# zero-savvy/vimz

Measured on AMD Instinct MI355X. Metric: nova_folding_steps_per_sec, higher is better.
Workload: dtype u32 limbs (256-bit Montgomery integers over BN254 Fr/Fq)

## Files before the change

### include/vimz_hip_testing.h

```cpp
#ifndef VIMZ_HIP_TESTING_H
#define VIMZ_HIP_TESTING_H
#include "vimz_hip.h"

#ifdef __cplusplus
extern "C" {
#endif

int vimz_cf_poke(vimz_cf* v, int which, size_t index, const uint64_t value[4]);
int vimz_cf_selfcheck(int steps, uint32_t* result, uint64_t counts[8]);
int64_t vimz_cf_selfcheck_last_step(int steps, void* buf, size_t cap);
int64_t vimz_cf_selfcheck_merge(int segs_run0, int segs_run1, void* buf, size_t cap);
int64_t vimz_worker_selftest(int jobs);
int vimz_strict_bits_selfcheck(int field, int values, uint64_t out[8]);
void vimz_test_forge_public_slot(int on);
int vimz_decider_selfcheck(int steps, int full, uint32_t* result, uint64_t counts[4]);
int vimz_testing_kzg_setup_seeded(vimz_ctx* ctx, const uint8_t* seed, size_t seed_len, size_t n, vimz_bases** srs_out, uint64_t vk_g2_out[16]);
int vimz_testing_decider_setup_seeded(vimz_cf* prover, const uint64_t kzg_vk_g2[16], int light, const uint8_t* seed, size_t seed_len, vimz_decider** out, double seconds[4]);

int vimz_test_fp29_probe(vimz_ctx* ctx, int field, int op, const uint32_t* a, const uint32_t* b, const uint32_t* c, const uint32_t* d, uint32_t* out, size_t n);
int vimz_test_spmv_cross16(vimz_ctx* ctx, const vimz_r1cs* S, size_t row0, size_t nrows, const vimz_vec* z, vimz_vec* az, vimz_vec* bz, vimz_vec* cz,
                           const vimz_vec* az1, const vimz_vec* bz1, const vimz_vec* cz1, const uint64_t u1[4], const uint64_t u2[4], int form, vimz_vec* T);
int vimz_test_cross_term_masked(vimz_ctx* ctx, size_t n, const vimz_vec* az1, const vimz_vec* bz1, const vimz_vec* cz1, const uint64_t u1[4], const vimz_vec* az2,
                                const vimz_vec* bz2, const vimz_vec* cz2, const uint64_t u2[4], int form, vimz_vec* T, vimz_vec* Tm, size_t nb);

#ifdef __cplusplus
}
#endif
#endif
```

### vimz_amd/csrc/image_hash.hip

```cpp
#include <hip/hip_runtime.h>
#include <algorithm>
#include <atomic>
#include <chrono>
#include <cstring>
#include <mutex>
#include <thread>
#include <vector>

#include "internal.hpp"
#include "fp29.hpp"
#include "circuit/poseidon_params.hpp"

using namespace vz;

namespace {

typedef Fp29<BnFr> F29;
constexpr int IH_STRIDE = 12;
constexpr int IH_WAVE = 64;
constexpr uint32_t IH_MAX_LEN = 1u << 20;

struct IhTables {
  const uint32_t* c[10]; const uint32_t* m[10]; const uint32_t* s[10]; const uint32_t* f[10];
  uint32_t rp[10];
};
struct IhImage { const uint8_t* px; const uint32_t* units; uint32_t h, w, ch, block, L, pad; };
struct IhSeg { uint32_t first_block, n_chains, chain_off, L; };
struct IhChain { uint32_t img, unit; };

__device__ __forceinline__ F29 ih_load29(const uint32_t* __restrict__ base, size_t idx) {
  const uint4* q = reinterpret_cast<const uint4*>(base + (size_t)IH_STRIDE * idx);
  const uint4 a = q[0], b = q[1], c = q[2];
  F29 r; r.v[0] = a.x; r.v[1] = a.y; r.v[2] = a.z; r.v[3] = a.w; r.v[4] = b.x; r.v[5] = b.y; r.v[6] = b.z; r.v[7] = b.w; r.v[8] = c.x;
  return r;
}
__device__ __forceinline__ F29 ih_shfl29(const F29& v, int src_lane) {
  F29 r;
#pragma unroll
  for (int k = 0; k < 9; k++) r.v[k] = __shfl(v.v[k], src_lane);
  return r;
}

__device__ __forceinline__ F29 ih_element(const IhImage& I, uint32_t unit, uint32_t e) {
  uint32_t w8[8] = {0, 0, 0, 0, 0, 0, 0, 0};
  if (I.units) {
    const uint4* q = reinterpret_cast<const uint4*>(I.units + 8 * ((size_t)unit * I.L + e));
    const uint4 a = q[0], b = q[1];
    w8[0] = a.x; w8[1] = a.y; w8[2] = a.z; w8[3] = a.w; w8[4] = b.x; w8[5] = b.y; w8[6] = b.z; w8[7] = b.w;
  } else {
    uint32_t row, col0, run;
    if (!I.block) {
      row = unit; col0 = e * 10; run = I.w - col0;
    } else {
      const uint32_t bw = (I.w + I.block - 1) / I.block, per_row = (I.block + 9) / 10;
      const uint32_t br = unit / bw, bc = unit % bw, r = e / per_row, c = e % per_row;
      row = br * I.block + r; col0 = bc * I.block + c * 10;
      const uint32_t end = min(I.w, (bc + 1) * I.block);
      run = row < I.h && col0 < end ? end - col0 : 0;
    }
    const uint32_t nc = I.ch < 3 ? I.ch : 3;
    const uint8_t* p = I.px + ((size_t)row * I.w + col0) * I.ch;
#pragma unroll
    for (uint32_t k = 0; k < 10; k++)
#pragma unroll
      for (uint32_t c = 0; c < 3; c++) {
        const uint32_t byte = 3 * k + c;
        if (k < run && c < nc) w8[byte >> 2] |= (uint32_t)p[(size_t)k * I.ch + c] << (8 * (byte & 3));
      }
  }
  F29 r2;
#pragma unroll
  for (int i = 0; i < 9; i++) r2.v[i] = F29::R2_29.l[i];
  return F29::mul(F29::pack(w8), r2);
}

template <int T>
__device__ __forceinline__ F29 ih_perm(const IhTables& P, F29 s, uint32_t li, int lane_base, int G) {
  const uint32_t* __restrict__ PC = P.c[T];
  const uint32_t* __restrict__ PM = P.m[T];
  const uint32_t* __restrict__ PS = P.s[T];
  const uint32_t* __restrict__ PF = P.f[T];
  const uint32_t rp = P.rp[T];
  const bool mine = li < (uint32_t)T;
  F29 Mrow[T];
#pragma unroll
  for (int j = 0; j < T; j++) Mrow[j] = mine ? ih_load29(PM, (size_t)li * T + j) : F29::zero();
  auto full_round = [&](uint32_t r) {
    if (mine) {
      s = F29::add(s, ih_load29(PC, (size_t)r * T + li));
      const F29 x2 = F29::sqr(s), x4 = F29::sqr(x2);
      s = F29::mul(x4, s);
    }
    F29 prod[T];
#pragma unroll
    for (int j = 0; j < T; j++) prod[j] = F29::mul(Mrow[j], ih_shfl29(s, lane_base + j));
#pragma unroll
    for (int stride = 1; stride < T; stride <<= 1)
#pragma unroll
      for (int j = 0; j + stride < T; j += 2 * stride) prod[j] = F29::add(prod[j], prod[j + stride]);
    s = prod[0].weak_reduce();
  };
  for (uint32_t r = 0; r < 4; r++) full_round(r);
  const bool l0 = li == 0;
  F29 ct = F29::zero(), rw = F29::zero(), cl = F29::zero();
  if (mine) { const size_t q = 3 * (size_t)li; ct = ih_load29(PS, q); rw = ih_load29(PS, q + 1); cl = ih_load29(PS, q + 2); }
  for (uint32_t r = 0; r < rp; r++) {
    F29 ctn = F29::zero(), rwn = F29::zero(), cln = F29::zero();
    if (mine && r + 1 < rp) { const size_t q = 3 * ((size_t)(r + 1) * T + li); ctn = ih_load29(PS, q); rwn = ih_load29(PS, q + 1); cln = ih_load29(PS, q + 2); }
    s = F29::add(s, ct);
    const F29 sl0 = ih_shfl29(s, lane_base);
    const F29 m1 = F29::mul(l0 ? s : rw, s);
    const F29 u = F29::mul(l0 ? rw : cl, sl0);
    F29 x4 = F29::zero();
    if (l0) x4 = F29::sqr(m1);
    const F29 x4b = ih_shfl29(x4, lane_base);
    const F29 m2 = F29::mul(x4b, u);
    F29 p = l0 ? m2 : (mine ? m1 : F29::zero());
    for (int off = G >> 1; off >= 1; off >>= 1) {
      F29 o;
#pragma unroll
      for (int k = 0; k < 9; k++) o.v[k] = __shfl_xor(p.v[k], off);
      p = F29::add(p, o);
    }
    s = (l0 ? p : (mine ? F29::add(s, m2) : s)).weak_reduce();
    ct = ctn; rw = rwn; cl = cln;
  }
  {
    F29 acc = F29::zero();
#pragma unroll
    for (int j = 0; j < T - 1; j++) {
      const F29 sj = ih_shfl29(s, lane_base + 1 + j);
      if (mine && !l0) acc = F29::add(acc, F29::mul(ih_load29(PF, (size_t)(li - 1) * (T - 1) + j), sj));
    }
    if (mine && !l0) s = acc.weak_reduce();
  }
  for (uint32_t r = 4 + rp; r < 8 + rp; r++) full_round(r);
  return s;
}

__global__ void __launch_bounds__(IH_WAVE) k_image_digests(IhTables P, const IhImage* __restrict__ imgs, const IhSeg* __restrict__ segs, uint32_t n_segs,
                                                           const IhChain* __restrict__ chains, uint32_t* __restrict__ out) {
  uint32_t sg = 0;
  while (sg + 1 < n_segs && blockIdx.x >= segs[sg + 1].first_block) sg++;
  const IhSeg S = segs[sg];
  const int G = S.L >= 8 ? 16 : 8;
  const uint32_t li = threadIdx.x & (uint32_t)(G - 1);
  const int lane_base = (int)(threadIdx.x & ~(uint32_t)(G - 1));
  const uint32_t k = (blockIdx.x - S.first_block) * (IH_WAVE / G) + threadIdx.x / G;
  const bool live = k < S.n_chains;
  const IhChain C = chains[S.chain_off + (live ? k : 0)];
  const IhImage I = imgs[C.img];
  const uint32_t L = S.L, rounds = (L + 7) / 8;
  F29 h = F29::zero();
  uint32_t done = 0;
  for (uint32_t r = 0; r < rounds; r++) {
    const uint32_t kin = r == 0 ? min(L, 8u) : min(L - done, 7u);
    const uint32_t t = r == 0 ? kin + 1 : kin + 2;
    F29 s = F29::zero();
    if (li >= 1 && li < t) s = (r > 0 && li == 1) ? h : ih_element(I, C.unit, done + li - (r == 0 ? 1 : 2));
    switch (t) {
      case 2: s = ih_perm<2>(P, s, li, lane_base, G); break;
      case 3: s = ih_perm<3>(P, s, li, lane_base, G); break;
      case 4: s = ih_perm<4>(P, s, li, lane_base, G); break;
      case 5: s = ih_perm<5>(P, s, li, lane_base, G); break;
      case 6: s = ih_perm<6>(P, s, li, lane_base, G); break;
      case 7: s = ih_perm<7>(P, s, li, lane_base, G); break;
      case 8: s = ih_perm<8>(P, s, li, lane_base, G); break;
      default: s = ih_perm<9>(P, s, li, lane_base, G); break;
    }
    h = ih_shfl29(s, lane_base);
    done += kin;
  }
  if (live && li == 0) {
    F29 one = F29::zero(); one.v[0] = 1;
    const F29 x = F29::mul(h, one).canon();
    uint32_t w8[8]; x.unpack(w8);
    uint4* o = reinterpret_cast<uint4*>(out + 8 * (size_t)k + 8 * (size_t)S.chain_off);
    o[0] = make_uint4(w8[0], w8[1], w8[2], w8[3]); o[1] = make_uint4(w8[4], w8[5], w8[6], w8[7]);
  }
}

struct IhHostTables { std::vector<uint32_t> words; size_t c[10], m[10], s[10], f[10]; uint32_t rp[10]; };
const IhHostTables& ih_host_tables() {
  static const IhHostTables T = [] {
    IhHostTables H{};
    auto put = [&](const std::vector<cb::Fe>& v) {
      const size_t at = H.words.size();
      H.words.resize(at + v.size() * (size_t)IH_STRIDE, 0u);
      for (size_t i = 0; i < v.size(); i++) { const F29 x = F29::from_std(v[i]); for (int k = 0; k < 9; k++) H.words[at + i * IH_STRIDE + k] = x.v[k]; }
      return at;
    };
    for (int t = 2; t <= 9; t++) {
      const cb::PoseidonTable& P = cb::poseidon_table(t);
      const auto& S = cb::poseidon_sparse_t<BnFr>(t);
      std::vector<cb::Fe> packed((size_t)P.rp * t * 3);
      for (int r = 0; r < P.rp; r++)
        for (int i = 0; i < t; i++) {
          cb::Fe* q = &packed[3 * ((size_t)r * t + i)];
          q[0] = S.ctil[(size_t)r * t + i]; q[1] = S.row[(size_t)r * t + i]; q[2] = i ? S.col[(size_t)r * (t - 1) + i - 1] : cb::Fe::zero();
        }
      H.c[t] = put(P.C); H.m[t] = put(P.M); H.s[t] = put(packed); H.f[t] = put(S.Pfin); H.rp[t] = (uint32_t)P.rp;
    }
    return H;
  }();
  return T;
}

inline size_t ih_align(size_t x) { return (x + 255) & ~(size_t)255; }

bool ih_below_modulus(const uint64_t* x) {
  const uint32_t* m = BnFr::MOD.w;
  for (int i = 3; i >= 0; i--) {
    const uint64_t mi = (uint64_t)m[2 * i] | (uint64_t)m[2 * i + 1] << 32;
    if (x[i] != mi) return x[i] < mi;
  }
  return false;
}

}

static int fail(vimz_ctx* c, int code, const char* what, hipError_t e = hipSuccess) { return vz::vz_fail(c, code, what, e); }

// ... 165 lines not shown
```

### vimz_amd/csrc/r1cs_capi.hip

```cpp
#include <hip/hip_runtime.h>
#include <array>
#include <cstring>
#include <memory>
#include <new>
#include <unordered_map>
#include <vector>

#include "internal.hpp"
#include "r1cs_ops.hpp"

using namespace vz;

struct vimz_r1cs {
  int field = 0;
  size_t nrows = 0, ncols = 0, nnz[3] = {0, 0, 0};
  CsrDev M[3] = {};
  uint32_t* dict = nullptr; size_t ndict = 0;
  uint32_t* long_items = nullptr; uint32_t n_long = 0, n_med = 0;
  uint32_t* scratch = nullptr;
  std::vector<void*> owned;
};

#define R_TRY(x) do { hipError_t _e = (x); if (_e != hipSuccess) return vz_fail(ctx, VIMZ_ERR_HIP, #x, _e); } while (0)

// ... 199 lines not shown
  uint32_t bad[2];
  R_TRY(hipMemcpyAsync(bad, bad_d, 8, hipMemcpyDeviceToHost, s));
  R_TRY(hipStreamSynchronize(s));
  *bad_rows = bad[0];
  if (first_bad) *first_bad = bad[0] ? bad[1] : ~0ull;
  return VIMZ_OK;
}

int vimz_vec_axpy(vimz_ctx* ctx, vimz_vec* x1, const uint64_t r[4], int form, const vimz_vec* x2, size_t n) {
  if (!ctx || !x1 || !x2 || !r) return vz_fail(ctx, VIMZ_ERR_INVALID, "vimz_vec_axpy: bad argument");
  if (x1->field != x2->field || n > x1->n || n > x2->n) return vz_fail(ctx, VIMZ_ERR_INVALID, "vimz_vec_axpy: fields differ or a vector is shorter than n");
  if (x1 == x2) return vz_fail(ctx, VIMZ_ERR_INVALID, "vimz_vec_axpy: x1 and x2 must be different vectors");
  if (!n) return VIMZ_OK;
  std::lock_guard<std::mutex> g(ctx->mu);
  R_TRY(hipSetDevice(ctx->device));
  int rc = field_dispatch(x1->field, [&](auto f) {
    typedef decltype(f) F;
    F a; memcpy(a.v, r, 32);
    if (!a.is_reduced()) return vz_fail(ctx, VIMZ_ERR_INVALID, "vimz_vec_axpy: r not below the modulus");
    if (form == VIMZ_FORM_CANONICAL) a = F::to_mont(a);
    hipLaunchKernelGGL(k_axpy_inplace<F>, dim3(stream_grid(n)), dim3(256), 0, ctx->stream, n, x1->d, a, (const uint32_t*)x2->d);
    return VIMZ_OK;
  });
  if (rc) return rc;
  R_TRY(hipGetLastError());
  return VIMZ_OK;
}

}

#ifdef VIMZ_TESTING
#include "../../include/vimz_hip_testing.h"
#include "fp29_probe.hpp"

namespace {
template <class P>
__global__ void __launch_bounds__(256) k_fp29_probe(int op, const uint32_t* __restrict__ a, const uint32_t* __restrict__ b, const uint32_t* __restrict__ c,
                                                    const uint32_t* __restrict__ d, uint32_t* __restrict__ out, size_t n) {
  VZ_GRID_STRIDE(i, n) {
    uint32_t x[4][FP29_PROBE_WORDS], r[FP29_PROBE_WORDS];
    for (int k = 0; k < FP29_PROBE_WORDS; k++) { x[0][k] = a[FP29_PROBE_WORDS * i + k]; x[1][k] = b[FP29_PROBE_WORDS * i + k]; x[2][k] = c[FP29_PROBE_WORDS * i + k]; x[3][k] = d[FP29_PROBE_WORDS * i + k]; }
    fp29_probe<P>(op, x[0], x[1], x[2], x[3], r);
    for (int k = 0; k < FP29_PROBE_WORDS; k++) out[FP29_PROBE_WORDS * i + k] = r[k];
  }
}
template <class F>
int scalar_arg(vimz_ctx* ctx, const uint64_t* u, int form, F* out, const char* what) {
  memcpy(out->v, u, 32);
  if (!out->is_reduced()) return vz_fail(ctx, VIMZ_ERR_INVALID, what);
  if (form == VIMZ_FORM_CANONICAL) *out = F::to_mont(*out);
  return VIMZ_OK;
}
}

extern "C" {

int vimz_test_fp29_probe(vimz_ctx* ctx, int field, int op, const uint32_t* a, const uint32_t* b, const uint32_t* c, const uint32_t* d, uint32_t* out, size_t n) {
  if (!ctx || !a || !b || !c || !d || !out || field < 0 || field > 3) return vz_fail(ctx, VIMZ_ERR_INVALID, "vimz_test_fp29_probe: bad argument");
  {
    uint32_t zero[FP29_PROBE_WORDS] = {}, r[FP29_PROBE_WORDS];
    if (fp29_probe<BnFr>(op, zero, zero, zero, zero, r)) return vz_fail(ctx, VIMZ_ERR_INVALID, "vimz_test_fp29_probe: unknown operation");
  }
  if (!n) return VIMZ_OK;
  std::lock_guard<std::mutex> g(ctx->mu);
  R_TRY(hipSetDevice(ctx->device));
  const size_t bytes = 4 * (size_t)FP29_PROBE_WORDS * n;
  uint32_t* buf = nullptr;
  R_TRY(hipMalloc((void**)&buf, 5 * bytes));
  const uint32_t* src[4] = {a, b, c, d};
  hipError_t e = hipSuccess;
  for (int k = 0; k < 4 && e == hipSuccess; k++) e = hipMemcpyAsync((char*)buf + k * bytes, src[k], bytes, hipMemcpyHostToDevice, ctx->stream);
  if (e == hipSuccess) {
    uint32_t* p = buf; const size_t w = (size_t)FP29_PROBE_WORDS * n;
    fp29_probe_field(field, [&](auto pp) {
      typedef decltype(pp) P;
      hipLaunchKernelGGL(k_fp29_probe<P>, dim3(stream_grid(n)), dim3(256), 0, ctx->stream, op, (const uint32_t*)p, (const uint32_t*)(p + w), (const uint32_t*)(p + 2 * w), (const uint32_t*)(p + 3 * w), p + 4 * w, n);
      return 0;
    });
    e = hipGetLastError();
  }
  if (e == hipSuccess) e = hipMemcpyAsync(out, (char*)buf + 4 * bytes, bytes, hipMemcpyDeviceToHost, ctx->stream);
  const hipError_t e2 = hipStreamSynchronize(ctx->stream);
  hipFree(buf);
  if (e != hipSuccess) return vz_fail(ctx, VIMZ_ERR_HIP, "vimz_test_fp29_probe", e);
  if (e2 != hipSuccess) return vz_fail(ctx, VIMZ_ERR_HIP, "vimz_test_fp29_probe: synchronize", e2);
  return VIMZ_OK;
}

int vimz_test_spmv_cross16(vimz_ctx* ctx, const vimz_r1cs* S, size_t row0, size_t nrows, const vimz_vec* z, vimz_vec* az, vimz_vec* bz, vimz_vec* cz,
                           const vimz_vec* az1, const vimz_vec* bz1, const vimz_vec* cz1, const uint64_t u1[4], const uint64_t u2[4], int form, vimz_vec* T) {
  if (!ctx || !S || !z || !az || !bz || !cz || !u1 || !u2) return vz_fail(ctx, VIMZ_ERR_INVALID, "vimz_test_spmv_cross16: bad argument");
  if (az1 && (!bz1 || !cz1 || !T)) return vz_fail(ctx, VIMZ_ERR_INVALID, "vimz_test_spmv_cross16: a running instance needs all of az1, bz1, cz1 and T");
  if (row0 > S->nrows || nrows > S->nrows - row0) return vz_fail(ctx, VIMZ_ERR_INVALID, "vimz_test_spmv_cross16: rows outside the shape");
  const vimz_vec* vs[7] = {az, bz, cz, az1, bz1, cz1, T};
  for (const vimz_vec* v : vs) if (v && (v->field != S->field || v->n < S->nrows)) return vz_fail(ctx, VIMZ_ERR_INVALID, "vimz_test_spmv_cross16: field or length of a vector does not fit the shape");
  if (z->field != S->field || z->n < S->ncols) return vz_fail(ctx, VIMZ_ERR_INVALID, "vimz_test_spmv_cross16: z does not fit the shape");
  if (!nrows) return VIMZ_OK;
  std::lock_guard<std::mutex> g(ctx->mu);
  R_TRY(hipSetDevice(ctx->device));
  int rc = field_dispatch(S->field, [&](auto f) {
    typedef decltype(f) F;
    F a, b; int r;
    if ((r = scalar_arg(ctx, u1, form, &a, "vimz_test_spmv_cross16: u1 not below the modulus")) || (r = scalar_arg(ctx, u2, form, &b, "vimz_test_spmv_cross16: u2 not below the modulus"))) return r;
    hipLaunchKernelGGL(k_spmv_cross16<F>, dim3((unsigned)((16 * nrows + 255) / 256)), dim3(256), 0, ctx->stream, S->M[0], S->M[1], S->M[2], (const uint32_t*)S->dict, (uint32_t)row0, (uint32_t)nrows,
                       (const uint32_t*)z->d, az->d, bz->d, cz->d, az1 ? (const uint32_t*)az1->d : (const uint32_t*)nullptr, bz1 ? (const uint32_t*)bz1->d : (const uint32_t*)nullptr,
                       cz1 ? (const uint32_t*)cz1->d : (const uint32_t*)nullptr, a, b, T ? T->d : (uint32_t*)nullptr);
    return VIMZ_OK;
  });
  if (rc) return rc;
  R_TRY(hipGetLastError());
  R_TRY(hipStreamSynchronize(ctx->stream));
  return VIMZ_OK;
}

int vimz_test_cross_term_masked(vimz_ctx* ctx, size_t n, const vimz_vec* az1, const vimz_vec* bz1, const vimz_vec* cz1, const uint64_t u1[4], const vimz_vec* az2, const vimz_vec* bz2,
                                const vimz_vec* cz2, const uint64_t u2[4], int form, vimz_vec* T, vimz_vec* Tm, size_t nb) {
  if (!ctx || !az1 || !bz1 || !cz1 || !az2 || !bz2 || !cz2 || !u1 || !u2 || !T) return vz_fail(ctx, VIMZ_ERR_INVALID, "vimz_test_cross_term_masked: bad argument");
  const vimz_vec* vs[8] = {az1, bz1, cz1, az2, bz2, cz2, T, Tm};
  for (const vimz_vec* v : vs) if (v && (v->field != T->field || v->n < n)) return vz_fail(ctx, VIMZ_ERR_INVALID, "vimz_test_cross_term_masked: field or length of a vector");
  if (nb > n || n >= (1ull << 32)) return vz_fail(ctx, VIMZ_ERR_INVALID, "vimz_test_cross_term_masked: nb beyond n");
  if (T == Tm) return vz_fail(ctx, VIMZ_ERR_INVALID, "vimz_test_cross_term_masked: T and Tm must differ");
// ... 20 lines not shown
```

### vimz_amd/csrc/witness.hpp

```cpp
#pragma once
#include <hip/hip_runtime.h>
#include "fp.hpp"
#include "fp29.hpp"
#include "circuit/program.hpp"
#include "vecops.hpp"

namespace vz {

typedef Fp<BnFr> Fr;

struct WitnessDev {
  const DecompGroup* decomp; uint32_t n_decomp;
  const LaneGroup* groups; uint32_t n_groups;
  const LaneInstr* instr;
  const LaneRow* rows;
  const HashJob* jobs; uint32_t n_jobs;
  const Chain* chains; uint32_t n_chains;
  const FieldOp* fops; uint32_t n_fops;
  const LcTerm* lc_terms; const uint32_t* dict;
  const uint32_t* pc3; const uint32_t* pm3;
  const uint32_t* pc9; const uint32_t* pm9;
  const uint32_t* ps3; const uint32_t* pf3;
  const uint32_t* ps9; const uint32_t* pf9;
  uint32_t rp3, rp9;
  const uint32_t *pc3_29, *pm3_29, *ps3_29, *pf3_29, *pc9_29, *pm9_29, *ps9_29, *pf9_29;
  uint32_t poseidon29;
  uint32_t n_wires, len_z, n_priv;
};

__device__ __forceinline__ Fr fr_from_small(long long v) {
  Fr x = Fr::zero();
  unsigned long long m = v < 0 ? (unsigned long long)(-v) : (unsigned long long)v;
  x.v[0] = (uint32_t)m; x.v[1] = (uint32_t)(m >> 32);
  x = Fr::to_mont(x);
  return v < 0 ? Fr::neg(x) : x;
}
// ... 200 lines not shown
    if (mine && r + 1 < rp) { const size_t q = 3 * ((size_t)(r + 1) * T + li); ctn = load_fe<Fr>(PS, q); rwn = load_fe<Fr>(PS, q + 1); cln = load_fe<Fr>(PS, q + 2); }
    s = Fr::add(s, ct);
    const Fr sl0 = shfl_fe(s, lane_base);
    const Fr m1 = Fr::mul(l0 ? s : rw, s);
    const Fr u = Fr::mul(l0 ? rw : cl, sl0);
    Fr x4 = Fr::zero();
    if (l0) { x4 = Fr::sqr(m1); if (live && Zrow) emit(nf0 + 3 * T + r, m1, x4, Fr::mul(x4, s)); }
    const Fr x4b = shfl_fe(x4, lane_base);
    const Fr m2 = Fr::mul(x4b, u);
    Fr p = l0 ? m2 : (mine ? m1 : Fr::zero());
#pragma unroll
    for (int off = 8; off >= 1; off >>= 1) {
      Fr o;
#pragma unroll
      for (int k = 0; k < 8; k++) o.v[k] = __shfl_xor(p.v[k], off);
      p = Fr::add(p, o);
    }
    s = l0 ? p : (mine ? Fr::add(s, m2) : s);
    ct = ctn; rw = rwn; cl = cln;
  }
  {
    Fr acc = Fr::zero();
#pragma unroll
    for (int j = 0; j < T - 1; j++) {
      const Fr sj = shfl_fe(s, lane_base + 1 + j);
      if (mine && !l0) acc = Fr::add(acc, Fr::mul(load_fe<Fr>(PF, (size_t)(li - 1) * (T - 1) + j), sj));
    }
    if (mine && !l0) s = acc;
  }
  for (uint32_t r = 4 + rp; r < R; r++) full_round(r);
  return s;
}

typedef Fp29<BnFr> F29;
constexpr int F29_STRIDE = 12;
__device__ __forceinline__ F29 load29(const uint32_t* __restrict__ base, size_t idx) {
  const uint4* q = reinterpret_cast<const uint4*>(base + (size_t)F29_STRIDE * idx);
  const uint4 a = q[0], b = q[1], c = q[2];
  F29 r; r.v[0] = a.x; r.v[1] = a.y; r.v[2] = a.z; r.v[3] = a.w; r.v[4] = b.x; r.v[5] = b.y; r.v[6] = b.z; r.v[7] = b.w; r.v[8] = c.x;
  return r;
}
__device__ __forceinline__ F29 shfl29(const F29& v, int src_lane) {
  F29 r;
#pragma unroll
  for (int k = 0; k < 9; k++) r.v[k] = __shfl(v.v[k], src_lane);
  return r;
}
static_assert(F29::KNUM == 169u, "the bounds in poseidon_group29 are written for BN254 Fr's quotient estimate");
__device__ __forceinline__ F29 weak_reduce29(const F29& a) { return a.weak_reduce(); }
__device__ __forceinline__ void store29_raw(uint32_t* __restrict__ Zrow, uint32_t wire, const F29& x) {
  uint32_t w[8]; x.unpack(w);
  uint4* q = reinterpret_cast<uint4*>(Zrow + 8 * (size_t)wire);
  q[0] = make_uint4(w[0], w[1], w[2], w[3]); q[1] = make_uint4(w[4], w[5], w[6], w[7]);
}

template <int T>
__device__ __forceinline__ F29 poseidon_group29(const WitnessDev& P, const HashJob& J, bool live, F29 s, bool in_const, uint32_t li, int lane_base,
                                                uint32_t* __restrict__ Zrow) {
  const uint32_t* PC = T == 3 ? P.pc3_29 : P.pc9_29;
  const uint32_t* PM = T == 3 ? P.pm3_29 : P.pm9_29;
  const uint32_t* PS = T == 3 ? P.ps3_29 : P.ps9_29;
  const uint32_t* PF = T == 3 ? P.pf3_29 : P.pf9_29;
  const uint32_t rp = T == 3 ? P.rp3 : P.rp9;
  const uint32_t R = 8 + rp;
  const bool mine = li < (uint32_t)T;
  F29 Mrow[T];
#pragma unroll
  for (int j = 0; j < T; j++) Mrow[j] = mine ? load29(PM, (size_t)li * T + j) : F29::zero();
  const unsigned long long nf_mask = __ballot(live && li >= 1 && mine && !in_const);
  const uint32_t grp_mask16 = (uint32_t)((nf_mask >> lane_base) & 0xffffull);
  const uint32_t nf_before = __popc(grp_mask16 & ((1u << li) - 1u));
  const uint32_t nf0 = __popc(grp_mask16);
  const uint32_t elim_slot = 3 * (nf0 + 3 * T + rp + 3 * T) + 2;
  const bool bound = J.out_wire != 0;
  auto emit = [&](uint32_t index, const F29& x2, const F29& x4, const F29& x5) {
    const uint32_t slot = 3 * index;
    auto wire_of = [&](uint32_t sl) { return J.wire_base + sl - ((bound && sl > elim_slot) ? 1u : 0u); };
    store29_raw(Zrow, wire_of(slot), x2);
    store29_raw(Zrow, wire_of(slot + 1), x4);
    if (!(bound && slot + 2 == elim_slot)) store29_raw(Zrow, wire_of(slot + 2), x5);
  };
  auto full_round = [&](uint32_t r) {
    if (mine) {
      s = F29::add(s, load29(PC, (size_t)r * T + li));
      const F29 x2 = F29::sqr(s), x4 = F29::sqr(x2), x5 = F29::mul(x4, s);
      const bool folded = r == 0 && in_const;
      if (live && !folded && Zrow) {
        uint32_t index;
        if (r == 0) index = nf_before;
        else if (r < 4) index = nf0 + (r - 1) * T + li;
        else index = nf0 + 3 * T + rp + (r - 4 - rp) * T + li;
        emit(index, x2, x4, x5);
      }
      s = x5;
    }
    F29 prod[T];
#pragma unroll
    for (int j = 0; j < T; j++) prod[j] = F29::mul(Mrow[j], shfl29(s, lane_base + j));
#pragma unroll
    for (int stride = 1; stride < T; stride <<= 1)
#pragma unroll
      for (int j = 0; j + stride < T; j += 2 * stride) prod[j] = F29::add(prod[j], prod[j + stride]);
    s = weak_reduce29(prod[0]);
  };
  for (uint32_t r = 0; r < 4; r++) full_round(r);
  const bool l0 = li == 0;
  F29 ct = F29::zero(), rw = F29::zero(), cl = F29::zero();
  if (mine) { const size_t q = 3 * (size_t)li; ct = load29(PS, q); rw = load29(PS, q + 1); cl = load29(PS, q + 2); }
  for (uint32_t r = 0; r < rp; r++) {
    F29 ctn = F29::zero(), rwn = F29::zero(), cln = F29::zero();
    if (mine && r + 1 < rp) { const size_t q = 3 * ((size_t)(r + 1) * T + li); ctn = load29(PS, q); rwn = load29(PS, q + 1); cln = load29(PS, q + 2); }
    s = F29::add(s, ct);
    const F29 sl0 = shfl29(s, lane_base);
    const F29 m1 = F29::mul(l0 ? s : rw, s);
    const F29 u = F29::mul(l0 ? rw : cl, sl0);
    F29 x4 = F29::zero();
    if (l0) { x4 = F29::sqr(m1); if (live && Zrow) emit(nf0 + 3 * T + r, m1, x4, F29::mul(x4, s)); }
    const F29 x4b = shfl29(x4, lane_base);
    const F29 m2 = F29::mul(x4b, u);
    F29 p = l0 ? m2 : (mine ? m1 : F29::zero());
#pragma unroll
    for (int off = 8; off >= 1; off >>= 1) {
      F29 o;
#pragma unroll
      for (int k = 0; k < 9; k++) o.v[k] = __shfl_xor(p.v[k], off);
      p = F29::add(p, o);
    }
    s = weak_reduce29(l0 ? p : (mine ? F29::add(s, m2) : s));
    ct = ctn; rw = rwn; cl = cln;
  }
  {
    F29 acc = F29::zero();
#pragma unroll
    for (int j = 0; j < T - 1; j++) {
      const F29 sj = shfl29(s, lane_base + 1 + j);
      if (mine && !l0) acc = F29::add(acc, F29::mul(load29(PF, (size_t)(li - 1) * (T - 1) + j), sj));
    }
    if (mine && !l0) s = weak_reduce29(acc);
  }
  for (uint32_t r = 4 + rp; r < R; r++) full_round(r);
  return s;
}

static __global__ void __launch_bounds__(64) k_wit_chains(WitnessDev P, uint32_t phase, uint32_t* __restrict__ Z, uint32_t* __restrict__ job_out,
                                                   const uint32_t* __restrict__ priv_rows) {
  const uint32_t row = blockIdx.y;
  const uint32_t sub = threadIdx.x >> 4, li = threadIdx.x & 15;
  const int lane_base = (int)(threadIdx.x & ~15u);
  uint32_t want = blockIdx.x * 4 + sub, seen = 0, cid = 0xffffffffu;
  for (uint32_t c = 0; c < P.n_chains; c++) if (P.chains[c].phase == phase) { if (seen == want) { cid = c; break; } seen++; }
  const bool active_chain = cid != 0xffffffffu;
  uint32_t* Zrow = priv_rows ? nullptr : Z + 8 * (size_t)row * P.n_wires;
  const uint32_t* prow = priv_rows ? priv_rows + 8 * (size_t)row * P.n_priv : nullptr;
  uint32_t* jrow = job_out + 8 * (size_t)row * (P.n_jobs + P.n_fops);
  const uint32_t njobs = active_chain ? P.chains[cid].job_cnt : 0;
  uint32_t max_jobs = njobs;
  for (int off = 32; off >= 16; off >>= 1) max_jobs = max(max_jobs, (uint32_t)__shfl_xor((int)max_jobs, off));
  Fr prev_out = Fr::zero();
  if (P.poseidon29) {
    F29 prev29 = F29::zero();
    for (uint32_t k = 0; k < max_jobs; k++) {
      const bool live = k < njobs;
      HashJob J;
      if (live) J = P.jobs[P.chains[cid].job_off + k]; else { J.t = 3; J.wire_base = 0; J.out_wire = 0; }
      const uint32_t t = J.t;
      F29 s = F29::zero();
      bool in_const = true;
      if (live && li >= 1 && li < t) {
        const ValRef ref = J.in[li - 1];
        in_const = ref.kind == REF_CONST_ZERO;
        if (ref.kind == REF_JOB && k > 0 && ref.idx == P.chains[cid].job_off + k - 1) s = prev29;
        else s = F29::from_std(wit_value(P, ref, Zrow, jrow, prow));
      }
      const bool any9 = __any(live && t == 9), any3 = __any(live && t != 9);
      F29 out = F29::zero();
      if (any9) { F29 o = poseidon_group29<9>(P, J, live && t == 9, s, in_const, li, lane_base, Zrow); if (t == 9) out = o; }
      if (any3) { F29 o = poseidon_group29<3>(P, J, live && t == 3, s, in_const, li, lane_base, Zrow); if (t != 9) out = o; }
      prev29 = shfl29(out, lane_base);
      if (live && li == 0) {
        const Fr o = out.to_std();
        store_fe(jrow, P.chains[cid].job_off + k, o);
        if (J.out_wire && Zrow) store_fe(Zrow, J.out_wire, o);
      }
    }
    return;
  }
  for (uint32_t k = 0; k < max_jobs; k++) {
    const bool live = k < njobs;
    HashJob J;
    if (live) J = P.jobs[P.chains[cid].job_off + k]; else { J.t = 3; J.wire_base = 0; J.out_wire = 0; }
    const uint32_t t = J.t;
    Fr s = Fr::zero();
    bool in_const = true;
    if (live && li >= 1 && li < t) {
      const ValRef ref = J.in[li - 1];
      in_const = ref.kind == REF_CONST_ZERO;
      if (ref.kind == REF_JOB && k > 0 && ref.idx == P.chains[cid].job_off + k - 1) s = prev_out;
      else s = wit_value(P, ref, Zrow, jrow, prow);
    }
    const bool any9 = __any(live && t == 9), any3 = __any(live && t != 9);
    Fr out = Fr::zero();
    if (any9) { Fr o = poseidon_group<9>(P, J, live && t == 9, s, in_const, li, lane_base, Zrow); if (t == 9) out = o; }
    if (any3) { Fr o = poseidon_group<3>(P, J, live && t == 3, s, in_const, li, lane_base, Zrow); if (t != 9) out = o; }
    prev_out = shfl_fe(out, lane_base);
    if (live && li == 0) {
      store_fe(jrow, P.chains[cid].job_off + k, out);
      if (J.out_wire && Zrow) store_fe(Zrow, J.out_wire, out);
    }
  }
}

// ... 75 lines not shown
```

Before: 1369.

## Share Poseidon29 permutation using DPP broadcasts and lazy-reduced dot products

Pulls the 29-bit-limb Poseidon permutation out of the image-hash and witness-chain kernels into one shared header. The MDS row products now accumulate in 64-bit columns and run a single Montgomery reduction per dot of up to six terms, where before each product was reduced separately. Lane broadcasts and group reductions use DPP row operations in place of ds_bpermute shuffles, and the group size is now a template parameter. The DPP control encodings (row_newbcast and similar) are tied to specific hardware and add correctness risk, and the partial-round emit path is restructured.

```diff
diff --git a/include/vimz_hip_testing.h b/include/vimz_hip_testing.h
--- a/include/vimz_hip_testing.h
+++ b/include/vimz_hip_testing.h
@@ -18,6 +18,7 @@
 int vimz_testing_decider_setup_seeded(vimz_cf* prover, const uint64_t kzg_vk_g2[16], int light, const uint8_t* seed, size_t seed_len, vimz_decider** out, double seconds[4]);
 
 int vimz_test_fp29_probe(vimz_ctx* ctx, int field, int op, const uint32_t* a, const uint32_t* b, const uint32_t* c, const uint32_t* d, uint32_t* out, size_t n);
+int vimz_test_fp29_dot(vimz_ctx* ctx, int field, int K, const uint32_t* xs, const uint32_t* ys, uint32_t* out, size_t n);
 int vimz_test_spmv_cross16(vimz_ctx* ctx, const vimz_r1cs* S, size_t row0, size_t nrows, const vimz_vec* z, vimz_vec* az, vimz_vec* bz, vimz_vec* cz,
                            const vimz_vec* az1, const vimz_vec* bz1, const vimz_vec* cz1, const uint64_t u1[4], const uint64_t u2[4], int form, vimz_vec* T);
 int vimz_test_cross_term_masked(vimz_ctx* ctx, size_t n, const vimz_vec* az1, const vimz_vec* bz1, const vimz_vec* cz1, const uint64_t u1[4], const vimz_vec* az2,
diff --git a/vimz_amd/csrc/image_hash.hip b/vimz_amd/csrc/image_hash.hip
--- a/vimz_amd/csrc/image_hash.hip
+++ b/vimz_amd/csrc/image_hash.hip
@@ -9,14 +9,13 @@
 
 #include "internal.hpp"
 #include "fp29.hpp"
+#include "poseidon29.hpp"
 #include "circuit/poseidon_params.hpp"
 
 using namespace vz;
 
 namespace {
 
-typedef Fp29<BnFr> F29;
-constexpr int IH_STRIDE = 12;
 constexpr int IH_WAVE = 64;
 constexpr uint32_t IH_MAX_LEN = 1u << 20;
 
@@ -27,19 +26,6 @@
 struct IhImage { const uint8_t* px; const uint32_t* units; uint32_t h, w, ch, block, L, pad; };
 struct IhSeg { uint32_t first_block, n_chains, chain_off, L; };
 struct IhChain { uint32_t img, unit; };
-
-__device__ __forceinline__ F29 ih_load29(const uint32_t* __restrict__ base, size_t idx) {
-  const uint4* q = reinterpret_cast<const uint4*>(base + (size_t)IH_STRIDE * idx);
-  const uint4 a = q[0], b = q[1], c = q[2];
-  F29 r; r.v[0] = a.x; r.v[1] = a.y; r.v[2] = a.z; r.v[3] = a.w; r.v[4] = b.x; r.v[5] = b.y; r.v[6] = b.z; r.v[7] = b.w; r.v[8] = c.x;
-  return r;
-}
-__device__ __forceinline__ F29 ih_shfl29(const F29& v, int src_lane) {
-  F29 r;
-#pragma unroll
-  for (int k = 0; k < 9; k++) r.v[k] = __shfl(v.v[k], src_lane);
-  return r;
-}
 
 __device__ __forceinline__ F29 ih_element(const IhImage& I, uint32_t unit, uint32_t e) {
   uint32_t w8[8] = {0, 0, 0, 0, 0, 0, 0, 0};
@@ -74,68 +60,9 @@
   return F29::mul(F29::pack(w8), r2);
 }
 
-template <int T>
-__device__ __forceinline__ F29 ih_perm(const IhTables& P, F29 s, uint32_t li, int lane_base, int G) {
-  const uint32_t* __restrict__ PC = P.c[T];
-  const uint32_t* __restrict__ PM = P.m[T];
-  const uint32_t* __restrict__ PS = P.s[T];
-  const uint32_t* __restrict__ PF = P.f[T];
-  const uint32_t rp = P.rp[T];
-  const bool mine = li < (uint32_t)T;
-  F29 Mrow[T];
-#pragma unroll
-  for (int j = 0; j < T; j++) Mrow[j] = mine ? ih_load29(PM, (size_t)li * T + j) : F29::zero();
-  auto full_round = [&](uint32_t r) {
-    if (mine) {
-      s = F29::add(s, ih_load29(PC, (size_t)r * T + li));
-      const F29 x2 = F29::sqr(s), x4 = F29::sqr(x2);
-      s = F29::mul(x4, s);
-    }
-    F29 prod[T];
-#pragma unroll
-    for (int j = 0; j < T; j++) prod[j] = F29::mul(Mrow[j], ih_shfl29(s, lane_base + j));
-#pragma unroll
-    for (int stride = 1; stride < T; stride <<= 1)
-#pragma unroll
-      for (int j = 0; j + stride < T; j += 2 * stride) prod[j] = F29::add(prod[j], prod[j + stride]);
-    s = prod[0].weak_reduce();
-  };
-  for (uint32_t r = 0; r < 4; r++) full_round(r);
-  const bool l0 = li == 0;
-  F29 ct = F29::zero(), rw = F29::zero(), cl = F29::zero();
-  if (mine) { const size_t q = 3 * (size_t)li; ct = ih_load29(PS, q); rw = ih_load29(PS, q + 1); cl = ih_load29(PS, q + 2); }
-  for (uint32_t r = 0; r < rp; r++) {
-    F29 ctn = F29::zero(), rwn = F29::zero(), cln = F29::zero();
-    if (mine && r + 1 < rp) { const size_t q = 3 * ((size_t)(r + 1) * T + li); ctn = ih_load29(PS, q); rwn = ih_load29(PS, q + 1); cln = ih_load29(PS, q + 2); }
-    s = F29::add(s, ct);
-    const F29 sl0 = ih_shfl29(s, lane_base);
-    const F29 m1 = F29::mul(l0 ? s : rw, s);
-    const F29 u = F29::mul(l0 ? rw : cl, sl0);
-    F29 x4 = F29::zero();
-    if (l0) x4 = F29::sqr(m1);
-    const F29 x4b = ih_shfl29(x4, lane_base);
-    const F29 m2 = F29::mul(x4b, u);
-    F29 p = l0 ? m2 : (mine ? m1 : F29::zero());
-    for (int off = G >> 1; off >= 1; off >>= 1) {
-      F29 o;
-#pragma unroll
-      for (int k = 0; k < 9; k++) o.v[k] = __shfl_xor(p.v[k], off);
-      p = F29::add(p, o);
-    }
-    s = (l0 ? p : (mine ? F29::add(s, m2) : s)).weak_reduce();
-    ct = ctn; rw = rwn; cl = cln;
-  }
-  {
-    F29 acc = F29::zero();
-#pragma unroll
-    for (int j = 0; j < T - 1; j++) {
-      const F29 sj = ih_shfl29(s, lane_base + 1 + j);
-      if (mine && !l0) acc = F29::add(acc, F29::mul(ih_load29(PF, (size_t)(li - 1) * (T - 1) + j), sj));
-    }
-    if (mine && !l0) s = acc.weak_reduce();
-  }
-  for (uint32_t r = 4 + rp; r < 8 + rp; r++) full_round(r);
-  return s;
+template <int G, int T>
+__device__ __forceinline__ F29 ih_perm(const IhTables& P, const F29& s, uint32_t li) {
+  return poseidon29_perm<G, T>(P29Tables{P.c[T], P.m[T], P.s[T], P.f[T], P.rp[T]}, s, li, P29NoEmit{});
 }
 
 __global__ void __launch_bounds__(IH_WAVE) k_image_digests(IhTables P, const IhImage* __restrict__ imgs, const IhSeg* __restrict__ segs, uint32_t n_segs,
@@ -145,7 +72,6 @@
   const IhSeg S = segs[sg];
   const int G = S.L >= 8 ? 16 : 8;
   const uint32_t li = threadIdx.x & (uint32_t)(G - 1);
-  const int lane_base = (int)(threadIdx.x & ~(uint32_t)(G - 1));
   const uint32_t k = (blockIdx.x - S.first_block) * (IH_WAVE / G) + threadIdx.x / G;
   const bool live = k < S.n_chains;
   const IhChain C = chains[S.chain_off + (live ? k : 0)];
@@ -158,17 +84,29 @@
     const uint32_t t = r == 0 ? kin + 1 : kin + 2;
     F29 s = F29::zero();
     if (li >= 1 && li < t) s = (r > 0 && li == 1) ? h : ih_element(I, C.unit, done + li - (r == 0 ? 1 : 2));
-    switch (t) {
-      case 2: s = ih_perm<2>(P, s, li, lane_base, G); break;
-      case 3: s = ih_perm<3>(P, s, li, lane_base, G); break;
-      case 4: s = ih_perm<4>(P, s, li, lane_base, G); break;
-      case 5: s = ih_perm<5>(P, s, li, lane_base, G); break;
-      case 6: s = ih_perm<6>(P, s, li, lane_base, G); break;
-      case 7: s = ih_perm<7>(P, s, li, lane_base, G); break;
-      case 8: s = ih_perm<8>(P, s, li, lane_base, G); break;
-      default: s = ih_perm<9>(P, s, li, lane_base, G); break;
-    }
-    h = ih_shfl29(s, lane_base);
+    if (G == 16) {
+      switch (t) {
+        case 3: s = ih_perm<16, 3>(P, s, li); break;
+        case 4: s = ih_perm<16, 4>(P, s, li); break;
+        case 5: s = ih_perm<16, 5>(P, s, li); break;
+        case 6: s = ih_perm<16, 6>(P, s, li); break;
+        case 7: s = ih_perm<16, 7>(P, s, li); break;
+        case 8: s = ih_perm<16, 8>(P, s, li); break;
+        default: s = ih_perm<16, 9>(P, s, li); break;
+      }
+      h = p29_bcast<16, 0>(s);
+    } else {
+      switch (t) {
+        case 2: s = ih_perm<8, 2>(P, s, li); break;
+        case 3: s = ih_perm<8, 3>(P, s, li); break;
+        case 4: s = ih_perm<8, 4>(P, s, li); break;
+        case 5: s = ih_perm<8, 5>(P, s, li); break;
+        case 6: s = ih_perm<8, 6>(P, s, li); break;
+        case 7: s = ih_perm<8, 7>(P, s, li); break;
+        default: s = ih_perm<8, 8>(P, s, li); break;
+      }
+      h = p29_bcast<8, 0>(s);
+    }
     done += kin;
   }
   if (live && li == 0) {
@@ -186,8 +124,8 @@
     IhHostTables H{};
     auto put = [&](const std::vector<cb::Fe>& v) {
       const size_t at = H.words.size();
-      H.words.resize(at + v.size() * (size_t)IH_STRIDE, 0u);
-      for (size_t i = 0; i < v.size(); i++) { const F29 x = F29::from_std(v[i]); for (int k = 0; k < 9; k++) H.words[at + i * IH_STRIDE + k] = x.v[k]; }
+      H.words.resize(at + v.size() * (size_t)F29_STRIDE, 0u);
+      for (size_t i = 0; i < v.size(); i++) { const F29 x = F29::from_std(v[i]); for (int k = 0; k < 9; k++) H.words[at + i * F29_STRIDE + k] = x.v[k]; }
       return at;
     };
     for (int t = 2; t <= 9; t++) {
diff --git a/vimz_amd/csrc/poseidon29.hpp b/vimz_amd/csrc/poseidon29.hpp
--- /dev/null
+++ b/vimz_amd/csrc/poseidon29.hpp
@@ -0,0 +1,142 @@
+#pragma once
+#include "fp29.hpp"
+
+namespace vz {
+
+template <int K, class P>
+VZ_HD Fp29<P> dot(const Fp29<P>* a, const Fp29<P>* b) {
+  static_assert(K >= 1 && K <= 6, "dot<K>: a 64-bit column holds 9K + 9 products below 2^58 plus carries only for K <= 6 (63·2^58 < 2^64)");
+  uint64_t acc[18];
+#pragma unroll
+  for (int k = 0; k < 18; k++) acc[k] = 0;
+#pragma unroll
+  for (int t = 0; t < K; t++)
+#pragma unroll
+    for (int i = 0; i < 9; i++)
+#pragma unroll
+      for (int j = 0; j < 9; j++) acc[i + j] += (uint64_t)a[t].v[i] * b[t].v[j];
+  return Fp29<P>::redc(acc);
+}
+
+#if defined(__HIPCC__)
+typedef Fp29<BnFr> F29;
+constexpr int F29_STRIDE = 12;
+static_assert(F29::KNUM == 169u, "the bounds in poseidon29_perm are written for BN254 Fr's quotient estimate (weak_reduce: below 1.9 p)");
+
+__device__ __forceinline__ F29 load29(const uint32_t* __restrict__ base, size_t idx) {
+  const uint4* q = reinterpret_cast<const uint4*>(base + (size_t)F29_STRIDE * idx);
+  const uint4 a = q[0], b = q[1], c = q[2];
+  F29 r; r.v[0] = a.x; r.v[1] = a.y; r.v[2] = a.z; r.v[3] = a.w; r.v[4] = b.x; r.v[5] = b.y; r.v[6] = b.z; r.v[7] = b.w; r.v[8] = c.x;
+  return r;
+}
+
+enum : int { P29_QUAD_XOR1 = 0xB1 , P29_QUAD_XOR2 = 0x4E , P29_HALF_MIRROR = 0x141, P29_ROR8 = 0x128,
+             P29_NEWBCAST = 0x150  };
+
+template <int G, int J>
+__device__ __forceinline__ F29 p29_bcast(const F29& v) {
+  static_assert((G == 8 || G == 16) && J >= 0 && J < G, "p29_bcast: lane J of a group of 8 or 16");
+  F29 r;
+#pragma unroll
+  for (int k = 0; k < 9; k++) {
+    if constexpr (G == 16) {
+      r.v[k] = (uint32_t)__builtin_amdgcn_update_dpp(0, (int)v.v[k], P29_NEWBCAST + J, 0xf, 0xf, true);
+    } else {
+      const int lo = __builtin_amdgcn_update_dpp(0, (int)v.v[k], P29_NEWBCAST + J, 0xf, 0x3, true);
+      r.v[k] = (uint32_t)__builtin_amdgcn_update_dpp(lo, (int)v.v[k], P29_NEWBCAST + 8 + J, 0xf, 0xc, false);
+    }
+  }
+  return r;
+}
+template <int CTRL>
+__device__ __forceinline__ F29 p29_add_dpp(const F29& p) {
+  F29 o;
+#pragma unroll
+  for (int k = 0; k < 9; k++) o.v[k] = (uint32_t)__builtin_amdgcn_update_dpp(0, (int)p.v[k], CTRL, 0xf, 0xf, true);
+  return F29::add(p, o);
+}
+template <int G, int T>
+__device__ __forceinline__ F29 p29_group_sum(F29 p) {
+  static_assert(T <= G, "p29_group_sum: the state does not fit the group");
+  if (T > 1) p = p29_add_dpp<P29_QUAD_XOR1>(p);
+  if (T > 2) p = p29_add_dpp<P29_QUAD_XOR2>(p);
+  if (T > 4) p = p29_add_dpp<P29_HALF_MIRROR>(p);
+  if (T > 8) p = p29_add_dpp<P29_ROR8>(p);
+  return p;
+}
+template <int G, int FIRST, int N, int J = 0>
+struct P29Gather {
+  static __device__ __forceinline__ void run(const F29& s, F29* g) { g[J] = p29_bcast<G, FIRST + J>(s); P29Gather<G, FIRST, N, J + 1>::run(s, g); }
+};
+template <int G, int FIRST, int N>
+struct P29Gather<G, FIRST, N, N> { static __device__ __forceinline__ void run(const F29&, F29*) {} };
+
+template <int N>
+__device__ __forceinline__ F29 p29_row_dot(const F29* a, const F29* b) {
+  static_assert(N >= 1 && N <= 12, "p29_row_dot: at most two dots of six terms");
+  if constexpr (N <= 6) return dot<N>(a, b);
+  else { constexpr int H = (N + 1) / 2; return F29::add(dot<H>(a, b), dot<N - H>(a + H, b + H)).weak_reduce(); }
+}
+
+struct P29Tables {
+  const uint32_t *c, *m, *s, *f;
+  uint32_t rp;
+};
+struct P29NoEmit { static constexpr bool on = false; };
+
+template <int G, int T, class E>
+__device__ __forceinline__ F29 poseidon29_perm(const P29Tables& P, F29 s, uint32_t li, const E& emit) {
+  static_assert(T >= 2 && T <= 9 && T <= G, "poseidon29_perm: widths 2..9, one lane per state element");
+  const uint32_t rp = P.rp;
+  const bool mine = li < (uint32_t)T, l0 = li == 0;
+  F29 Mrow[T];
+#pragma unroll
+  for (int j = 0; j < T; j++) Mrow[j] = mine ? load29(P.m, (size_t)li * T + j) : F29::zero();
+  auto full_round = [&](uint32_t r) {
+    if (mine) {
+      s = F29::add(s, load29(P.c, (size_t)r * T + li));
+      const F29 x2 = F29::sqr(s), x4 = F29::sqr(x2), x5 = F29::mul(x4, s);
+      if constexpr (E::on) emit.full(r, x2, x4, x5);
+      s = x5;
+    }
+    F29 g[T];
+    P29Gather<G, 0, T>::run(s, g);
+    s = p29_row_dot<T>(Mrow, g);
+  };
+  for (uint32_t r = 0; r < 4; r++) full_round(r);
+  F29 ct = F29::zero(), rw = F29::zero(), cl = F29::zero();
+  if (mine) { const size_t q = 3 * (size_t)li; ct = load29(P.s, q); rw = load29(P.s, q + 1); cl = load29(P.s, q + 2); }
+  for (uint32_t r = 0; r < rp; r++) {
+    F29 ctn = F29::zero(), rwn = F29::zero(), cln = F29::zero();
+    if (mine && r + 1 < rp) { const size_t q = 3 * ((size_t)(r + 1) * T + li); ctn = load29(P.s, q); rwn = load29(P.s, q + 1); cln = load29(P.s, q + 2); }
+    s = F29::add(s, ct);
+    const F29 m1 = F29::mul(l0 ? s : rw, s);
+    F29 m2;
+    if constexpr (E::on) {
+      F29 x5 = F29::zero();
+      if (l0) { const F29 x4 = F29::sqr(m1); x5 = F29::mul(x4, s); emit.partial(r, m1, x4, x5); }
+      m2 = F29::mul(l0 ? rw : cl, p29_bcast<G, 0>(x5));
+    } else {
+      const F29 u = F29::mul(l0 ? rw : cl, p29_bcast<G, 0>(s));
+      F29 x4 = F29::zero();
+      if (l0) x4 = F29::sqr(m1);
+      m2 = F29::mul(p29_bcast<G, 0>(x4), u);
+    }
+    const F29 p = p29_group_sum<G, T>(l0 ? m2 : (mine ? m1 : F29::zero()));
+    s = (l0 ? p : (mine ? F29::add(s, m2) : s)).weak_reduce();
+    ct = ctn; rw = rwn; cl = cln;
+  }
+  {
+    F29 Frow[T - 1], g[T - 1];
+#pragma unroll
+    for (int j = 0; j < T - 1; j++) Frow[j] = (mine && !l0) ? load29(P.f, (size_t)(li - 1) * (T - 1) + j) : F29::zero();
+    P29Gather<G, 1, T - 1>::run(s, g);
+    const F29 b = p29_row_dot<T - 1>(Frow, g);
+    if (mine && !l0) s = b;
+  }
+  for (uint32_t r = 4 + rp; r < 8 + rp; r++) full_round(r);
+  return s;
+}
+#endif
+
+}
diff --git a/vimz_amd/csrc/r1cs_capi.hip b/vimz_amd/csrc/r1cs_capi.hip
--- a/vimz_amd/csrc/r1cs_capi.hip
+++ b/vimz_amd/csrc/r1cs_capi.hip
@@ -255,6 +255,7 @@
 #ifdef VIMZ_TESTING
 #include "../../include/vimz_hip_testing.h"
 #include "fp29_probe.hpp"
+#include "poseidon29.hpp"
 
 namespace {
 template <class P>
@@ -265,6 +266,27 @@
     for (int k = 0; k < FP29_PROBE_WORDS; k++) { x[0][k] = a[FP29_PROBE_WORDS * i + k]; x[1][k] = b[FP29_PROBE_WORDS * i + k]; x[2][k] = c[FP29_PROBE_WORDS * i + k]; x[3][k] = d[FP29_PROBE_WORDS * i + k]; }
     fp29_probe<P>(op, x[0], x[1], x[2], x[3], r);
     for (int k = 0; k < FP29_PROBE_WORDS; k++) out[FP29_PROBE_WORDS * i + k] = r[k];
+  }
+}
+template <class P, int K>
+__global__ void __launch_bounds__(256) k_fp29_dot(const uint32_t* __restrict__ xs, const uint32_t* __restrict__ ys, uint32_t* __restrict__ out, size_t n) {
+  VZ_GRID_STRIDE(i, n) {
+    Fp29<P> a[K], b[K];
+    for (int t = 0; t < K; t++)
+      for (int k = 0; k < 9; k++) { a[t].v[k] = xs[9 * ((size_t)K * i + t) + k]; b[t].v[k] = ys[9 * ((size_t)K * i + t) + k]; }
+    const Fp29<P> r = dot<K>(a, b);
+    for (int k = 0; k < 9; k++) out[9 * i + k] = r.v[k];
+  }
+}
+template <class P>
+void launch_fp29_dot(int K, unsigned grid, hipStream_t st, const uint32_t* xs, const uint32_t* ys, uint32_t* out, size_t n) {
+  switch (K) {
+    case 1: hipLaunchKernelGGL((k_fp29_dot<P, 1>), dim3(grid), dim3(256), 0, st, xs, ys, out, n); break;
+    case 2: hipLaunchKernelGGL((k_fp29_dot<P, 2>), dim3(grid), dim3(256), 0, st, xs, ys, out, n); break;
+    case 3: hipLaunchKernelGGL((k_fp29_dot<P, 3>), dim3(grid), dim3(256), 0, st, xs, ys, out, n); break;
+    case 4: hipLaunchKernelGGL((k_fp29_dot<P, 4>), dim3(grid), dim3(256), 0, st, xs, ys, out, n); break;
+    case 5: hipLaunchKernelGGL((k_fp29_dot<P, 5>), dim3(grid), dim3(256), 0, st, xs, ys, out, n); break;
+    default: hipLaunchKernelGGL((k_fp29_dot<P, 6>), dim3(grid), dim3(256), 0, st, xs, ys, out, n); break;
   }
 }
 template <class F>
@@ -310,6 +332,32 @@
   return VIMZ_OK;
 }
 
+int vimz_test_fp29_dot(vimz_ctx* ctx, int field, int K, const uint32_t* xs, const uint32_t* ys, uint32_t* out, size_t n) {
+  if (!ctx || !xs || !ys || !out || field < 0 || field > 3 || K < 1 || K > 6 || n > (1u << 24))
+    return vz_fail(ctx, VIMZ_ERR_INVALID, "vimz_test_fp29_dot: bad argument (fields 0..3, K 1..6, at most 2^24 cases)");
+  if (!n) return VIMZ_OK;
+  std::lock_guard<std::mutex> g(ctx->mu);
+  R_TRY(hipSetDevice(ctx->device));
+  const size_t in_bytes = 4 * 9 * (size_t)K * n, out_bytes = 4 * 9 * n;
+  char* buf = nullptr;
+  R_TRY(hipMalloc((void**)&buf, 2 * in_bytes + out_bytes));
+  hipError_t e = hipMemcpyAsync(buf, xs, in_bytes, hipMemcpyHostToDevice, ctx->stream);
+  if (e == hipSuccess) e = hipMemcpyAsync(buf + in_bytes, ys, in_bytes, hipMemcpyHostToDevice, ctx->stream);
+  if (e == hipSuccess) {
+    fp29_probe_field(field, [&](auto pp) {
+      launch_fp29_dot<decltype(pp)>(K, stream_grid(n), ctx->stream, (const uint32_t*)buf, (const uint32_t*)(buf + in_bytes), (uint32_t*)(buf + 2 * in_bytes), n);
+      return 0;
+    });
+    e = hipGetLastError();
+  }
+  if (e == hipSuccess) e = hipMemcpyAsync(out, buf + 2 * in_bytes, out_bytes, hipMemcpyDeviceToHost, ctx->stream);
+  const hipError_t e2 = hipStreamSynchronize(ctx->stream);
+  hipFree(buf);
+  if (e != hipSuccess) return vz_fail(ctx, VIMZ_ERR_HIP, "vimz_test_fp29_dot", e);
+  if (e2 != hipSuccess) return vz_fail(ctx, VIMZ_ERR_HIP, "vimz_test_fp29_dot: synchronize", e2);
+  return VIMZ_OK;
+}
+
 int vimz_test_spmv_cross16(vimz_ctx* ctx, const vimz_r1cs* S, size_t row0, size_t nrows, const vimz_vec* z, vimz_vec* az, vimz_vec* bz, vimz_vec* cz,
                            const vimz_vec* az1, const vimz_vec* bz1, const vimz_vec* cz1, const uint64_t u1[4], const uint64_t u2[4], int form, vimz_vec* T) {
   if (!ctx || !S || !z || !az || !bz || !cz || !u1 || !u2) return vz_fail(ctx, VIMZ_ERR_INVALID, "vimz_test_spmv_cross16: bad argument");
diff --git a/vimz_amd/csrc/witness.hpp b/vimz_amd/csrc/witness.hpp
--- a/vimz_amd/csrc/witness.hpp
+++ b/vimz_amd/csrc/witness.hpp
@@ -2,6 +2,7 @@
 #include <hip/hip_runtime.h>
 #include "fp.hpp"
 #include "fp29.hpp"
+#include "poseidon29.hpp"
 #include "circuit/program.hpp"
 #include "vecops.hpp"
 
@@ -268,114 +269,47 @@
   return s;
 }
 
-typedef Fp29<BnFr> F29;
-constexpr int F29_STRIDE = 12;
-__device__ __forceinline__ F29 load29(const uint32_t* __restrict__ base, size_t idx) {
-  const uint4* q = reinterpret_cast<const uint4*>(base + (size_t)F29_STRIDE * idx);
-  const uint4 a = q[0], b = q[1], c = q[2];
-  F29 r; r.v[0] = a.x; r.v[1] = a.y; r.v[2] = a.z; r.v[3] = a.w; r.v[4] = b.x; r.v[5] = b.y; r.v[6] = b.z; r.v[7] = b.w; r.v[8] = c.x;
-  return r;
-}
-__device__ __forceinline__ F29 shfl29(const F29& v, int src_lane) {
-  F29 r;
-#pragma unroll
-  for (int k = 0; k < 9; k++) r.v[k] = __shfl(v.v[k], src_lane);
-  return r;
-}
-static_assert(F29::KNUM == 169u, "the bounds in poseidon_group29 are written for BN254 Fr's quotient estimate");
-__device__ __forceinline__ F29 weak_reduce29(const F29& a) { return a.weak_reduce(); }
 __device__ __forceinline__ void store29_raw(uint32_t* __restrict__ Zrow, uint32_t wire, const F29& x) {
   uint32_t w[8]; x.unpack(w);
   uint4* q = reinterpret_cast<uint4*>(Zrow + 8 * (size_t)wire);
   q[0] = make_uint4(w[0], w[1], w[2], w[3]); q[1] = make_uint4(w[4], w[5], w[6], w[7]);
 }
 
-template <int T>
-__device__ __forceinline__ F29 poseidon_group29(const WitnessDev& P, const HashJob& J, bool live, F29 s, bool in_const, uint32_t li, int lane_base,
-                                                uint32_t* __restrict__ Zrow) {
-  const uint32_t* PC = T == 3 ? P.pc3_29 : P.pc9_29;
-  const uint32_t* PM = T == 3 ? P.pm3_29 : P.pm9_29;
-  const uint32_t* PS = T == 3 ? P.ps3_29 : P.ps9_29;
-  const uint32_t* PF = T == 3 ? P.pf3_29 : P.pf9_29;
-  const uint32_t rp = T == 3 ? P.rp3 : P.rp9;
-  const uint32_t R = 8 + rp;
-  const bool mine = li < (uint32_t)T;
-  F29 Mrow[T];
-#pragma unroll
-  for (int j = 0; j < T; j++) Mrow[j] = mine ? load29(PM, (size_t)li * T + j) : F29::zero();
-  const unsigned long long nf_mask = __ballot(live && li >= 1 && mine && !in_const);
-  const uint32_t grp_mask16 = (uint32_t)((nf_mask >> lane_base) & 0xffffull);
-  const uint32_t nf_before = __popc(grp_mask16 & ((1u << li) - 1u));
-  const uint32_t nf0 = __popc(grp_mask16);
-  const uint32_t elim_slot = 3 * (nf0 + 3 * T + rp + 3 * T) + 2;
-  const bool bound = J.out_wire != 0;
-  auto emit = [&](uint32_t index, const F29& x2, const F29& x4, const F29& x5) {
+struct ChainWires29 {
+  static constexpr bool on = true;
+  uint32_t* Zrow; uint32_t wire_base, elim_slot, nf_before, nf0, T, rp, li; bool bound, live, in_const;
+  __device__ __forceinline__ void put(uint32_t index, const F29& x2, const F29& x4, const F29& x5) const {
     const uint32_t slot = 3 * index;
-    auto wire_of = [&](uint32_t sl) { return J.wire_base + sl - ((bound && sl > elim_slot) ? 1u : 0u); };
+    auto wire_of = [&](uint32_t sl) { return wire_base + sl - ((bound && sl > elim_slot) ? 1u : 0u); };
     store29_raw(Zrow, wire_of(slot), x2);
     store29_raw(Zrow, wire_of(slot + 1), x4);
     if (!(bound && slot + 2 == elim_slot)) store29_raw(Zrow, wire_of(slot + 2), x5);
-  };
-  auto full_round = [&](uint32_t r) {
-    if (mine) {
-      s = F29::add(s, load29(PC, (size_t)r * T + li));
-      const F29 x2 = F29::sqr(s), x4 = F29::sqr(x2), x5 = F29::mul(x4, s);
-      const bool folded = r == 0 && in_const;
-      if (live && !folded && Zrow) {
-        uint32_t index;
-        if (r == 0) index = nf_before;
-        else if (r < 4) index = nf0 + (r - 1) * T + li;
-        else index = nf0 + 3 * T + rp + (r - 4 - rp) * T + li;
-        emit(index, x2, x4, x5);
-      }
-      s = x5;
-    }
-    F29 prod[T];
-#pragma unroll
-    for (int j = 0; j < T; j++) prod[j] = F29::mul(Mrow[j], shfl29(s, lane_base + j));
-#pragma unroll
-    for (int stride = 1; stride < T; stride <<= 1)
-#pragma unroll
-      for (int j = 0; j + stride < T; j += 2 * stride) prod[j] = F29::add(prod[j], prod[j + stride]);
-    s = weak_reduce29(prod[0]);
-  };
-  for (uint32_t r = 0; r < 4; r++) full_round(r);
-  const bool l0 = li == 0;
-  F29 ct = F29::zero(), rw = F29::zero(), cl = F29::zero();
-  if (mine) { const size_t q = 3 * (size_t)li; ct = load29(PS, q); rw = load29(PS, q + 1); cl = load29(PS, q + 2); }
-  for (uint32_t r = 0; r < rp; r++) {
-    F29 ctn = F29::zero(), rwn = F29::zero(), cln = F29::zero();
-    if (mine && r + 1 < rp) { const size_t q = 3 * ((size_t)(r + 1) * T + li); ctn = load29(PS, q); rwn = load29(PS, q + 1); cln = load29(PS, q + 2); }
-    s = F29::add(s, ct);
-    const F29 sl0 = shfl29(s, lane_base);
-    const F29 m1 = F29::mul(l0 ? s : rw, s);
-    const F29 u = F29::mul(l0 ? rw : cl, sl0);
-    F29 x4 = F29::zero();
-    if (l0) { x4 = F29::sqr(m1); if (live && Zrow) emit(nf0 + 3 * T + r, m1, x4, F29::mul(x4, s)); }
-    const F29 x4b = shfl29(x4, lane_base);
-    const F29 m2 = F29::mul(x4b, u);
-    F29 p = l0 ? m2 : (mine ? m1 : F29::zero());
-#pragma unroll
-    for (int off = 8; off >= 1; off >>= 1) {
-      F29 o;
-#pragma unroll
-      for (int k = 0; k < 9; k++) o.v[k] = __shfl_xor(p.v[k], off);
-      p = F29::add(p, o);
-    }
-    s = weak_reduce29(l0 ? p : (mine ? F29::add(s, m2) : s));
-    ct = ctn; rw = rwn; cl = cln;
-  }
-  {
-    F29 acc = F29::zero();
-#pragma unroll
-    for (int j = 0; j < T - 1; j++) {
-      const F29 sj = shfl29(s, lane_base + 1 + j);
-      if (mine && !l0) acc = F29::add(acc, F29::mul(load29(PF, (size_t)(li - 1) * (T - 1) + j), sj));
-    }
-    if (mine && !l0) s = weak_reduce29(acc);
-  }
-  for (uint32_t r = 4 + rp; r < R; r++) full_round(r);
-  return s;
+  }
+  __device__ __forceinline__ void full(uint32_t r, const F29& x2, const F29& x4, const F29& x5) const {
+    if (!live || (r == 0 && in_const)) return;
+    uint32_t index;
+    if (r == 0) index = nf_before;
+    else if (r < 4) index = nf0 + (r - 1) * T + li;
+    else index = nf0 + 3 * T + rp + (r - 4 - rp) * T + li;
+    put(index, x2, x4, x5);
+  }
+  __device__ __forceinline__ void partial(uint32_t r, const F29& x2, const F29& x4, const F29& x5) const { if (live) put(nf0 + 3 * T + r, x2, x4, x5); }
+};
+
+template <int T>
+__device__ __forceinline__ F29 poseidon_chain29(const WitnessDev& P, const HashJob& J, bool live, F29 s, bool in_const, uint32_t li, int lane_base,
+                                                uint32_t* __restrict__ Zrow) {
+  const P29Tables tab = T == 3 ? P29Tables{P.pc3_29, P.pm3_29, P.ps3_29, P.pf3_29, P.rp3} : P29Tables{P.pc9_29, P.pm9_29, P.ps9_29, P.pf9_29, P.rp9};
+  if (!Zrow) return poseidon29_perm<16, T>(tab, s, li, P29NoEmit{});
+  const bool mine = li < (uint32_t)T;
+  const unsigned long long nf_mask = __ballot(live && li >= 1 && mine && !in_const);
+  const uint32_t grp_mask16 = (uint32_t)((nf_mask >> lane_base) & 0xffffull);
+  ChainWires29 W;
+  W.Zrow = Zrow; W.wire_base = J.wire_base; W.T = T; W.rp = tab.rp; W.li = li; W.bound = J.out_wire != 0; W.live = live; W.in_const = in_const;
+  W.nf_before = __popc(grp_mask16 & ((1u << li) - 1u));
+  W.nf0 = __popc(grp_mask16);
+  W.elim_slot = 3 * (W.nf0 + 3 * T + tab.rp + 3 * T) + 2;
+  return poseidon29_perm<16, T>(tab, s, li, W);
 }
 
 static __global__ void __launch_bounds__(64) k_wit_chains(WitnessDev P, uint32_t phase, uint32_t* __restrict__ Z, uint32_t* __restrict__ job_out,
@@ -410,9 +344,9 @@
       }
       const bool any9 = __any(live && t == 9), any3 = __any(live && t != 9);
       F29 out = F29::zero();
-      if (any9) { F29 o = poseidon_group29<9>(P, J, live && t == 9, s, in_const, li, lane_base, Zrow); if (t == 9) out = o; }
-      if (any3) { F29 o = poseidon_group29<3>(P, J, live && t == 3, s, in_const, li, lane_base, Zrow); if (t != 9) out = o; }
-      prev29 = shfl29(out, lane_base);
+      if (any9) { F29 o = poseidon_chain29<9>(P, J, live && t == 9, s, in_const, li, lane_base, Zrow); if (t == 9) out = o; }
+      if (any3) { F29 o = poseidon_chain29<3>(P, J, live && t == 3, s, in_const, li, lane_base, Zrow); if (t != 9) out = o; }
+      prev29 = p29_bcast<16, 0>(out);
       if (live && li == 0) {
         const Fr o = out.to_std();
         store_fe(jrow, P.chains[cid].job_off + k, o);
```

New measurement: 1372, median of 4. No clear change (+0.3%).
